# E3SM-Project/tinman_sandbox

Hardware: AMD Instinct MI355X
Metric: element-RHS-updates/sec (node) + achieved HBM GB/s, NP=4 NLEV=72 fp64 (higher is better)
Workload: dtype f64

## Files before the change

include/caar_tuning.h:

```cpp
#ifndef CAAR_TUNING_H
#define CAAR_TUNING_H

#include "caar.h"

#ifdef __cplusplus
extern "C" {
#endif

const char *caar_kernel_name(int np, int nlev);
int caar_num_variants(int np, int nlev);
int caar_select_variant(int np, int nlev, int variant);
int caar_selected_variant(int np, int nlev);
const char *caar_variant_info(int np, int nlev, int variant);
int caar_set_xcd_chunked(int on);
#define CAAR_CACHE_WINDOW_DEFAULT (224LL << 20)
int caar_set_cache_window(long long bytes);
long long caar_get_cache_window(void);
int caar_set_adaptive_window(int on);
int caar_get_adaptive_window(void);
long long caar_adaptive_window_lock_count(void);
int caar_adaptive_window_state(const double *vn0_dev, double *ms_window, double *ms_streaming, long long *probes);
int caar_adaptive_window_reset(void);


long long caar_context_cache_window(CaarContext *ctx);

int caar_set_fused_steps(int on);
int caar_get_fused_steps(void);
int caar_has_fused_steps(int np, int nlev, int variant);

enum { CAAR_PLACE_DEFAULT = 0, CAAR_PLACE_SPREAD = 1, CAAR_PLACE_MALLOC = 2 };
#define CAAR_PLACEMENT_POOL_DEFAULT (128LL << 30)
typedef struct CaarPlacement {
  int policy;
  long long pool_bytes;
  double max_free_fraction;
} CaarPlacement;
int caar_arrays_alloc_ex(CaarArena **arena, const CaarDims *dims, int device, const CaarPlacement *placement,
                         CaarArrays *out_dev);
int caar_arrays_placement(const CaarArena *arena, long long *pool_chunks, long long *chunk_bytes);

int caar_create_ex(CaarContext **ctx, const CaarDims *dims, int device, const CaarPlacement *placement);

int caar_stream_copy(double *dst_dev, const double *src_dev, long long n_doubles, int lane_bytes,
                     void *stream);
int caar_stream_copy_tuned(double *dst_dev, const double *src_dev, long long n_doubles, int variant,
                           void *stream);
int caar_stream_copy_tuned_variants(void);
const char *caar_stream_copy_tuned_info(int variant);
int caar_traffic_skeleton(const CaarDims *dims, const CaarArrays *dev, const CaarParams *params,
// ... 15 lines not shown
```

tinman_sandbox_amd/caar.py:

```python
import ctypes as C
import math
import os

import numpy as np
import torch

_HERE = os.path.dirname(os.path.abspath(__file__))
LIB_PATH = os.path.join(_HERE, "csrc", {"debug": "libcaar_hip_debug.so", "extra": "libcaar_hip_extra.so"}.get(
    os.environ.get("CAAR_LIBRARY", ""), "libcaar_hip.so"))
if os.environ.get("CAAR_LIBRARY_PATH"):
    LIB_PATH = os.environ["CAAR_LIBRARY_PATH"]

ARRAY_NAMES = (
    "elem_D", "elem_Dinv", "elem_fcor", "elem_spheremp", "elem_metdet", "elem_rmetdet",
    "elem_state_dp3d", "elem_state_v", "elem_state_T", "elem_state_phis", "elem_state_Qdp",
    "elem_derived_eta_dot_dpdn", "elem_derived_omega_p", "elem_derived_phi",
    "elem_derived_pecnd", "elem_derived_vn0",
)
MUTATED = ("elem_state_dp3d", "elem_state_v", "elem_state_T", "elem_derived_eta_dot_dpdn",
           "elem_derived_omega_p", "elem_derived_phi", "elem_derived_vn0")

_dp = C.POINTER(C.c_double)


# ... 33 lines not shown
class _CaarOperatorGeometry(C.Structure):
    _fields_ = [(n, C.c_void_p) for n in ("D", "Dinv", "metdet", "rmetdet", "spheremp", "mp", "metinv", "tensorVisc",
                                           "vec_sph2cart")]


class _CaarOperatorScalars(C.Structure):
    _fields_ = [("rrearth", C.c_double), ("alpha", C.c_double), ("beta", C.c_double), ("nu_ratio", C.c_double)]


SPHERE_OPERATORS = {
    "gradient_sphere": (0, False, True), "divergence_sphere": (1, True, False), "vorticity_sphere": (2, True, False),
    "divergence_sphere_wk": (3, True, False), "laplace_simple": (4, False, False), "laplace_tensor": (5, False, False),
    "curl_sphere_wk_testcov": (6, False, True), "grad_sphere_wk_testcov": (7, False, True),
    "vlaplace_sphere_wk_contra": (8, True, True), "vlaplace_sphere_wk_cartesian": (9, True, True),
    "gradient_sphere_update": (10, False, True), "divergence_sphere_update": (11, True, False),
    "vlaplace_sphere_wk_cartesian_damped": (12, True, True),
    "laplace_tensor_replace": (13, False, False),
}


class CaarLibrary:

    BOUNDARY_SYMBOLS = (
        "caar_supported", "caar_supported_ex", "caar_abi_version", "caar_device_count", "caar_strerror", "caar_array_len",
        "caar_algorithmic_bytes", "caar_launch", "caar_launch_steps", "caar_sphere_operator", "caar_sphere_operator_range",
        "caar_sphere_operator_ex", "caar_euler_step", "caar_preq_hydrostatic", "caar_preq_omega_ps", "caar_sphere_operator_host",
        "caar_preq_hydrostatic_host", "caar_preq_omega_ps_host", "caar_launch_state_norms", "caar_layout_from_f90",
        "caar_layout_to_f90", "caar_arrays_alloc", "caar_arrays_free", "caar_create", "caar_destroy", "caar_upload",
        "caar_download", "caar_upload_f90", "caar_download_f90", "caar_upload_f90_arrays", "caar_run", "caar_run_steps",
        "caar_sync", "caar_device_arrays", "caar_stream", "caar_state_norms", "caar_map_host", "caar_run_mapped",
        "caar_unmap_host")
    TUNING_SYMBOLS = (
        "caar_kernel_name", "caar_num_variants", "caar_select_variant", "caar_selected_variant", "caar_variant_info",
        "caar_set_xcd_chunked", "caar_set_cache_window", "caar_get_cache_window", "caar_set_adaptive_window",
        "caar_get_adaptive_window", "caar_adaptive_window_state", "caar_adaptive_window_reset", "caar_adaptive_window_lock_count",
        "caar_context_cache_window",
        "caar_set_fused_steps", "caar_get_fused_steps", "caar_has_fused_steps", "caar_arrays_alloc_ex",
        "caar_arrays_placement", "caar_create_ex", "caar_stream_copy", "caar_stream_copy_tuned",
        "caar_stream_copy_tuned_variants", "caar_stream_copy_tuned_info", "caar_traffic_skeleton", "caar_time_runs",
        "caar_reciprocal", "caar_debug_dp3d_violations")
    F90_SYMBOLS = ("caar_launch_f90", "caar_launch_steps_f90")
    DSS_SYMBOLS = ("caar_dss_plan_create", "caar_dss_plan_destroy", "caar_dss_plan_info", "caar_dss_launch")
    SYMBOLS = BOUNDARY_SYMBOLS + TUNING_SYMBOLS + F90_SYMBOLS + DSS_SYMBOLS

    def __init__(self, path=LIB_PATH):
        if not os.path.exists(path):
            raise CaarError(
                "HIP extension %s is missing: build it with `python -m tinman_sandbox_amd.build` "
                "(there is no CPU fallback)" % path)
        L = self.lib = C.CDLL(path)
        for s in self.SYMBOLS:
            getattr(L, s)
        vp = C.c_void_p
        L.caar_supported.argtypes = [C.c_int, C.c_int]
        L.caar_supported_ex.argtypes = [C.c_int, C.c_int, C.c_int]
        L.caar_debug_dp3d_violations.argtypes = [C.c_int]
        L.caar_debug_dp3d_violations.restype = C.c_longlong
        L.caar_strerror.argtypes = [C.c_int]
        L.caar_strerror.restype = C.c_char_p
        L.caar_array_len.argtypes = [C.POINTER(_CaarDims), C.c_int]
        L.caar_array_len.restype = C.c_longlong
        L.caar_algorithmic_bytes.argtypes = [C.c_int, C.c_int, C.c_int]
        L.caar_algorithmic_bytes.restype = C.c_longlong
        L.caar_launch.argtypes = [C.POINTER(_CaarDims), C.POINTER(_CaarArrays), vp,
                                  C.POINTER(_CaarParams), vp]
        L.caar_launch_steps.argtypes = [C.POINTER(_CaarDims), C.POINTER(_CaarArrays), vp, C.POINTER(_CaarParams), C.c_int,
                                        C.c_int, vp]
        L.caar_launch_f90.argtypes = [C.POINTER(_CaarDims), C.POINTER(_CaarArrays), vp, C.POINTER(_CaarParams), vp]
        L.caar_launch_steps_f90.argtypes = [C.POINTER(_CaarDims), C.POINTER(_CaarArrays), vp, C.POINTER(_CaarParams), C.c_int,
                                            C.c_int, vp]
        L.caar_launch_state_norms.argtypes = [C.POINTER(_CaarDims), C.POINTER(_CaarArrays), C.c_int,
                                              C.c_int, C.c_int, vp, vp]
        L.caar_sphere_operator.argtypes = [C.POINTER(_CaarDims), C.POINTER(_CaarArrays), vp, C.c_int, C.c_int,
                                           C.c_int, vp, vp, C.c_double, vp]
        L.caar_sphere_operator_range.argtypes = [C.POINTER(_CaarDims), C.POINTER(_CaarArrays), vp, C.c_int, C.c_int,
                                                 C.c_int, C.c_int, vp, vp, C.c_double, vp]
        L.caar_euler_step.argtypes = [C.POINTER(_CaarDims), C.POINTER(_CaarOperatorGeometry), vp, C.c_int, C.c_int, C.c_int,
                                      C.c_int, C.c_double, C.c_double, vp, vp, vp, vp]
        L.caar_sphere_operator_ex.argtypes = [C.POINTER(_CaarDims), C.POINTER(_CaarOperatorGeometry), vp, C.c_int, C.c_int,
                                              C.c_int, C.c_int, vp, vp, C.POINTER(_CaarOperatorScalars), vp]
        L.caar_preq_hydrostatic.argtypes = [C.POINTER(_CaarDims), C.c_int, vp, vp, vp, vp, C.c_double, vp, vp]
        L.caar_preq_omega_ps.argtypes = [C.POINTER(_CaarDims), C.c_int, vp, vp, vp, vp, vp]
        L.caar_sphere_operator_host.argtypes = [C.POINTER(_CaarDims), C.POINTER(_CaarArrays), vp, C.c_int, C.c_int, vp, vp,
                                                C.c_double]
        L.caar_preq_hydrostatic_host.argtypes = [C.POINTER(_CaarDims), vp, vp, vp, vp, C.c_double, vp]
        L.caar_preq_omega_ps_host.argtypes = [C.POINTER(_CaarDims), vp, vp, vp, vp]
        L.caar_reciprocal.argtypes = [vp, vp, C.c_longlong, vp]
        L.caar_kernel_name.argtypes = [C.c_int, C.c_int]
        L.caar_kernel_name.restype = C.c_char_p
        L.caar_num_variants.argtypes = [C.c_int, C.c_int]
        L.caar_select_variant.argtypes = [C.c_int, C.c_int, C.c_int]
        L.caar_variant_info.argtypes = [C.c_int, C.c_int, C.c_int]
        L.caar_variant_info.restype = C.c_char_p
        L.caar_set_xcd_chunked.argtypes = [C.c_int]
        L.caar_set_cache_window.argtypes = [C.c_longlong]
        L.caar_get_cache_window.restype = C.c_longlong
        L.caar_adaptive_window_state.argtypes = [vp, C.POINTER(C.c_double), C.POINTER(C.c_double), C.POINTER(C.c_longlong)]
        L.caar_adaptive_window_lock_count.restype = C.c_longlong
        L.caar_context_cache_window.argtypes = [vp]
        L.caar_context_cache_window.restype = C.c_longlong
        L.caar_selected_variant.argtypes = [C.c_int, C.c_int]
        L.caar_layout_from_f90.argtypes = [C.POINTER(_CaarDims), C.POINTER(_CaarArrays),
                                           C.POINTER(_CaarArrays), C.c_int, C.c_int, vp]
        L.caar_layout_to_f90.argtypes = [C.POINTER(_CaarDims), C.POINTER(_CaarArrays),
                                         C.POINTER(_CaarArrays), C.c_int, C.c_int, C.c_int, vp]
        L.caar_stream_copy.argtypes = [vp, vp, C.c_longlong, C.c_int, vp]
        L.caar_stream_copy_tuned.argtypes = [vp, vp, C.c_longlong, C.c_int, vp]
        L.caar_stream_copy_tuned_info.argtypes = [C.c_int]
        L.caar_stream_copy_tuned_info.restype = C.c_char_p
        L.caar_traffic_skeleton.argtypes = [C.POINTER(_CaarDims), C.POINTER(_CaarArrays),
                                            C.POINTER(_CaarParams), C.c_int, vp]
        L.caar_arrays_alloc.argtypes = [C.POINTER(vp), C.POINTER(_CaarDims), C.c_int, C.POINTER(_CaarArrays)]
        L.caar_arrays_alloc_ex.argtypes = [C.POINTER(vp), C.POINTER(_CaarDims), C.c_int, C.POINTER(_CaarPlacement),
                                           C.POINTER(_CaarArrays)]
        L.caar_arrays_free.argtypes = [vp]
        L.caar_arrays_placement.argtypes = [vp, C.POINTER(C.c_longlong), C.POINTER(C.c_longlong)]
        L.caar_create.argtypes = [C.POINTER(vp), C.POINTER(_CaarDims), C.c_int]
        L.caar_create_ex.argtypes = [C.POINTER(vp), C.POINTER(_CaarDims), C.c_int, C.POINTER(_CaarPlacement)]
        L.caar_destroy.argtypes = [vp]
        L.caar_destroy.restype = None
        L.caar_upload.argtypes = [vp, C.POINTER(_CaarArrays), C.c_int, C.c_int]
        L.caar_download.argtypes = [vp, C.POINTER(_CaarArrays), C.c_int, C.c_int, C.c_int]
        L.caar_upload_f90.argtypes = [vp, C.POINTER(_CaarArrays), C.c_int, C.c_int]
        L.caar_upload_f90_arrays.argtypes = [vp, C.POINTER(_CaarArrays), C.c_int, C.c_int, C.c_uint]
        L.caar_download_f90.argtypes = [vp, C.POINTER(_CaarArrays), C.c_int, C.c_int, C.c_int]
        L.caar_run.argtypes = [vp, C.POINTER(_CaarParams)]
        L.caar_sync.argtypes = [vp]
        L.caar_device_arrays.argtypes = [vp, C.POINTER(_CaarArrays)]
        L.caar_stream.argtypes = [vp]
# ... 594 lines not shown
```

tinman_sandbox_amd/csrc/caar_abi.hip:

```cpp
#include <hip/hip_runtime.h>

#include <atomic>
#include <cstdio>
#include <cstring>
#include <mutex>
#include <new>
#include <vector>

#include "../../include/caar.h"
#include "../../include/caar_f90.h"
#include "../../include/caar_tuning.h"
#include "caar_kernel_args.h"
#include "caar_window_tuner.h"

namespace caar {
extern KernelVariant kNp4Nlev72[];
extern int kNp4Nlev72Count;
extern KernelVariant kNp4Nlev128[];
extern int kNp4Nlev128Count;
extern KernelVariant kNp8Nlev72[];
extern int kNp8Nlev72Count;
#if CAAR_EXTRA_NLEV
extern KernelVariant kNp4Nlev32[], kNp4Nlev60[], kNp4Nlev64[], kNp4Nlev80[], kNp4Nlev96[], kNp4Nlev26[], kNp4Nlev30[];
extern int kNp4Nlev32Count, kNp4Nlev60Count, kNp4Nlev64Count, kNp4Nlev80Count, kNp4Nlev96Count, kNp4Nlev26Count, kNp4Nlev30Count;
// ... 81 lines not shown
  }
  void destroy() {
    if (dev) (void)hipFree(dev);
    delete host;
    dev = nullptr;
    host = nullptr;
  }
  hipError_t sync(const CaarDims& d, CaarParams* p, hipStream_t stream, const double** dvv_dev) {
    const size_t n = (size_t)d.np * d.np;
    if (!dvv_valid || std::memcmp(host->data(), p->Dvv, sizeof(double) * n) != 0) {
      std::memcpy(host->data(), p->Dvv, sizeof(double) * n);
      hipError_t e = hipMemcpyAsync(dev, host->data(), sizeof(double) * n, hipMemcpyHostToDevice, stream);
      if (e != hipSuccess) return e;
      dvv_valid = true;
    }
    if (p->rsplit == 0) {
      const size_t m = (size_t)d.nlev + 1;
      if (!hybi_valid || std::memcmp(host->data() + 64, p->hybi, sizeof(double) * m) != 0) {
        std::memcpy(host->data() + 64, p->hybi, sizeof(double) * m);
        hipError_t e = hipMemcpyAsync(dev + 64, host->data() + 64, sizeof(double) * m, hipMemcpyHostToDevice, stream);
        if (e != hipSuccess) return e;
        hybi_valid = true;
      }
      p->hybi_dev = dev + 64;
    }
    *dvv_dev = dev;
    return hipSuccess;
  }
};
}

static std::atomic<int> g_xcd_chunked{-1};
static std::atomic<long long> g_cache_window{CAAR_CACHE_WINDOW_DEFAULT};
static std::atomic<int> g_fused_steps{1};

namespace caar {
struct LaunchChoice {
  int variant;
  int xcd_chunked;
  long long cache_window;
  bool adapted;
};
static LaunchChoice launch_choice(const Config* cfg) {
  LaunchChoice c;
  c.variant = cfg ? cfg->selected.load(std::memory_order_relaxed) : 0;
  c.xcd_chunked = g_xcd_chunked.load(std::memory_order_relaxed);
  if (c.xcd_chunked < 0) c.xcd_chunked = cfg && cfg->variants[c.variant].prefers_xcd_chunked ? 1 : 0;
  c.cache_window = g_cache_window.load(std::memory_order_relaxed);
  c.adapted = false;
  return c;
}
}

namespace caar {
struct WindowTuner {
  std::atomic<const void*> key{nullptr};
  std::atomic<int> device{-1};
  std::atomic<int> use_window{1};
  std::atomic<long long> idle{0};
  WindowTunerState st;
  long long last_use = 0;
  hipEvent_t ev[WindowTunerState::kSlots] = {};

  void restart(const void* k, int dev) {
    key.store(nullptr, std::memory_order_relaxed);
    st.reset();
    last_use = 0;
    use_window.store(1, std::memory_order_relaxed);
    idle.store(0, std::memory_order_relaxed);
    device.store(dev, std::memory_order_relaxed);
    key.store(k, std::memory_order_release);
  }
};
struct HipStampBackend {
  WindowTuner* t;
  hipStream_t stream;
  bool stamp(int slot) {
    hipEvent_t& e = t->ev[slot];
    if (!e && hipEventCreate(&e) != hipSuccess) e = nullptr;
    return e && hipEventRecord(e, stream) == hipSuccess;
  }
// ... 150 lines not shown
  return (c->nlev != 0 || nlev <= 128 || CAAR_EXTRA_NLEV) ? 1 : 0;
}

const char* caar_kernel_name(int np, int nlev) {
  const caar::Config* c = caar::find_config(np, nlev);
  return c ? c->variants[c->selected.load()].kernel : nullptr;
}

int caar_num_variants(int np, int nlev) {
  const caar::Config* c = caar::find_config(np, nlev);
  return c ? c->count : 0;
}

int caar_select_variant(int np, int nlev, int variant) {
  caar::Config* c = caar::find_config(np, nlev);
  if (!c) return CAAR_EUNSUPPORTED;
  if (variant < 0 || variant >= c->count) return CAAR_EINVAL;
  c->selected.store(variant);
  return CAAR_OK;
}

int caar_selected_variant(int np, int nlev) {
  const caar::Config* c = caar::find_config(np, nlev);
  return c ? c->selected.load() : CAAR_EUNSUPPORTED;
}

int caar_set_cache_window(long long bytes) {
  if (bytes < 0) return CAAR_EINVAL;
  g_cache_window.store(bytes);
  return CAAR_OK;
}

long long caar_get_cache_window(void) { return g_cache_window.load(); }

int caar_set_adaptive_window(int on) {
  g_adaptive_window.store(on ? 1 : 0);
  return CAAR_OK;
}
int caar_get_adaptive_window(void) { return g_adaptive_window.load(); }

int caar_adaptive_window_state(const double* vn0_dev, double* ms_window, double* ms_streaming, long long* probes) {
  caar::WindowTuners* all = caar::window_tuners();
  std::lock_guard<std::mutex> g(all->mu);
  for (auto& t : all->t)
    if (vn0_dev && t.key.load(std::memory_order_relaxed) == (const void*)vn0_dev) {
      if (ms_window) *ms_window = t.st.ms_window;
      if (ms_streaming) *ms_streaming = t.st.ms_streaming;
      if (probes) *probes = t.st.probes;
      return t.use_window.load(std::memory_order_relaxed);
    }
  return -1;
}

long long caar_adaptive_window_lock_count(void) { return caar::window_tuners()->locked_calls.load(std::memory_order_relaxed); }

int caar_adaptive_window_reset(void) {
  caar::WindowTuners* all = caar::window_tuners();
  std::lock_guard<std::mutex> g(all->mu);
  for (auto& t : all->t) t.restart(nullptr, -1);
  return CAAR_OK;
}

int caar_set_fused_steps(int on) {
  g_fused_steps.store(on ? 1 : 0);
  return CAAR_OK;
}
// ... 562 lines not shown
  if (!out || !dims || dims->num_elems <= 0) return CAAR_EINVAL;
  if (!caar::find_config(dims->np, dims->nlev)) return CAAR_EUNSUPPORTED;
  int ndev = 0;
  if (hipGetDeviceCount(&ndev) != hipSuccess || ndev <= 0) return CAAR_ENODEVICE;
  if (device < 0 || device >= ndev) return CAAR_EINVAL;
  HIP_TRY(hipSetDevice(device));
  CaarContext* c = new (std::nothrow) CaarContext();
  if (!c) return CAAR_ENOMEM;
  std::memset(c, 0, sizeof(*c));
  c->dims = *dims;
  c->device = device;
  hipError_t e = hipStreamCreateWithFlags(&c->stream, hipStreamNonBlocking);
  if (e == hipSuccess) {
    const int rc = caar_arrays_alloc_ex(&c->arena, dims, device, placement, &c->dev);
    if (rc != CAAR_OK) {
      caar_destroy(c);
      return rc;
    }
  }
  if (e == hipSuccess) e = c->consts.create(dims->nlev);
  if (e == hipSuccess) e = hipMalloc((void**)&c->norms_dev, sizeof(double) * 3 * dims->num_elems);
  if (e != hipSuccess) {
    caar_destroy(c);
    return e == hipErrorOutOfMemory ? CAAR_ENOMEM : (int)e;
  }
  caar::device_shares_add(device, caar::keepable_bytes(c->dims));
  c->shares_registered = true;
  *out = c;
  return CAAR_OK;
}

long long caar_context_cache_window(CaarContext* c) {
  if (!c) return -1;
  return caar::device_share_of(c->device, c->dims, g_cache_window.load(std::memory_order_relaxed));
}

void caar_destroy(CaarContext* c) {
  if (!c) return;
  if (c->shares_registered) caar::device_shares_add(c->device, -caar::keepable_bytes(c->dims));
  int caller_dev = -1;
  if (hipGetDevice(&caller_dev) != hipSuccess) caller_dev = -1;
  (void)hipSetDevice(c->device);
  if (c->stream) (void)hipStreamSynchronize(c->stream);
  if (c->arena) (void)caar_arrays_free(c->arena);
  c->consts.destroy();
  if (c->norms_dev) (void)hipFree(c->norms_dev);
  if (c->stage_dev) (void)hipFree(c->stage_dev);
  if (c->steps_exec) (void)hipGraphExecDestroy(c->steps_exec);
  delete c->steps_hybi;
  if (c->stream) (void)hipStreamDestroy(c->stream);
  if (caller_dev >= 0 && caller_dev != c->device) (void)hipSetDevice(caller_dev);
  delete c;
}

static int copy_range(CaarContext* c, const CaarArrays* host, int i, int e0, int e1, bool to_device) {
  const long long per = caar_array_len(&c->dims, i) / c->dims.num_elems;
  double* h = *array_slot(host, i);
  double* d = *array_slot(&c->dev, i);
  if (!h) return CAAR_EINVAL;
  const size_t off = (size_t)per * e0, bytes = sizeof(double) * (size_t)per * (e1 - e0);
  if (to_device) HIP_TRY(hipMemcpyAsync(d + off, h + off, bytes, hipMemcpyHostToDevice, c->stream));
  else HIP_TRY(hipMemcpyAsync(h + off, d + off, bytes, hipMemcpyDeviceToHost, c->stream));
  return CAAR_OK;
}

int caar_upload(CaarContext* c, const CaarArrays* host, int e0, int e1) {
  if (!c || !host || e0 < 0 || e1 > c->dims.num_elems || e0 > e1) return CAAR_EINVAL;
// ... 302 lines not shown
```

tinman_sandbox_amd/csrc/caar_dss.hip:

```cpp
#include <hip/hip_runtime.h>

#include <algorithm>
#include <climits>
#include <cstdlib>
#include <new>
#include <utility>
#include <vector>

#include "../../include/caar_dss.h"

#pragma clang fp contract(off)

namespace caar {

constexpr int kDssThreads = 256;
constexpr int kDssLdsBytes = 32768;

__host__ __device__ constexpr int dss_bp_a(int np, int bp) {
  return bp < np ? 0 : (bp < np + 2 * (np - 2) ? 1 + (bp - np) / 2 : np - 1);
}
__host__ __device__ constexpr int dss_bp_b(int np, int bp) {
  return bp < np ? bp : (bp < np + 2 * (np - 2) ? (((bp - np) & 1) ? np - 1 : 0) : bp - np - 2 * (np - 2));
}
__host__ __device__ constexpr int dss_bp_of(int np, int a, int b) {
  return a == 0 ? b
                : (a == np - 1 ? np + 2 * (np - 2) + b
                               : (b == 0 ? np + 2 * (a - 1) : (b == np - 1 ? np + 2 * (a - 1) + 1 : -1)));
}

struct DssArgs {
  double* T;
  double* v;
  double* dp;
  const double* rsph;
  double* edge;
  const int* sharers;
  long long tstride;
  int nlev;
  int num_elems;
  int kc;
  int ldsw;
};

__device__ inline long long dss_element(int num_elems) {
  const int per = (num_elems + 7) / 8;
  const long long e = (long long)(blockIdx.x % 8) * per + blockIdx.x / 8;
  return e < num_elems ? e : -1;
}

template <int NP, bool F90>
__device__ inline double* dss_slab_value(const DssArgs& g, long long e, int k, int s, int& f, int& a, int& b) {
  constexpr int PP = NP * NP;
  const long long lev = e * g.tstride + (long long)k * PP;
  if (s < PP || s >= 3 * PP) {
    const int o = s < PP ? s : s - 3 * PP;
    f = s < PP ? 0 : 3;
    a = F90 ? o % NP : o / NP;
    b = F90 ? o / NP : o % NP;
    return (s < PP ? g.T : g.dp) + lev + o;
  }
  const int o = s - PP;
  int c, q;
  if (F90) {
    c = o / PP;
    q = o % PP;
    b = q / NP;
    a = q % NP;
  } else {
    c = o & 1;
    q = o >> 1;
    a = q / NP;
    b = q % NP;
  }
  f = 1 + c;
  return g.v + 2 * lev + o;
}

template <int NP, bool F90>
__device__ inline const double* dss_point(const DssArgs& g, long long e, int k, int f, int a, int b) {
  constexpr int PP = NP * NP;
  const long long lev = e * g.tstride + (long long)k * PP;
  const int p = F90 ? b * NP + a : a * NP + b;
  if (f == 0) return g.T + lev + p;
  if (f == 3) return g.dp + lev + p;
  return g.v + 2 * lev + (F90 ? (f - 1) * PP + p : 2 * p + (f - 1));
}

template <int NP, bool F90>
__global__ __launch_bounds__(kDssThreads) void caar_dss_pack(const DssArgs g) {
  constexpr int NB = 4 * (NP - 1);
  extern __shared__ double lds[];
  const long long e = dss_element(g.num_elems);
  if (e < 0) return;
  const int lane = threadIdx.x & 63, w = __builtin_amdgcn_readfirstlane(threadIdx.x >> 6);
  const int row4 = 4 * g.nlev, ldsw = g.ldsw;
  double* erow = g.edge + e * NB * row4;
  for (int k0 = 0; k0 < g.nlev; k0 += g.kc) {
    const int kc = min(g.kc, g.nlev - k0), n = kc * 4 * NB, m = 4 * kc;
#pragma unroll 4
    for (int i = threadIdx.x; i < n; i += kDssThreads) {
      const int kk = i / (4 * NB), r = i % (4 * NB), f = r / NB, bp = r % NB;
      lds[bp * ldsw + f * kc + kk] = *dss_point<NP, F90>(g, e, k0 + kk, f, dss_bp_a(NP, bp), dss_bp_b(NP, bp));
    }
    __syncthreads();
    for (int bp = w; bp < NB; bp += 4)
      for (int t = lane; t < m; t += 64) {
        const int f = t / kc;
        erow[bp * row4 + f * g.nlev + k0 + (t - f * kc)] = lds[bp * ldsw + t];
      }
    __syncthreads();
  }
}

template <int NP, bool F90>
__global__ __launch_bounds__(kDssThreads) void caar_dss_unpack(const DssArgs g) {
  constexpr int NB = 4 * (NP - 1), PP = NP * NP, MS = CAAR_DSS_MAX_SHARERS, BATCH = 8;
  extern __shared__ double lds[];
  const long long e = dss_element(g.num_elems);
  if (e < 0) return;
  const int lane = threadIdx.x & 63, w = __builtin_amdgcn_readfirstlane(threadIdx.x >> 6);
  const int row4 = 4 * g.nlev, ldsw = g.ldsw;
  const double* rsph = g.rsph + e * PP;
  for (int k0 = 0; k0 < g.nlev; k0 += g.kc) {
    const int kc = min(g.kc, g.nlev - k0), m = 4 * kc;
    for (int bp = w; bp < NB; bp += 4) {
      const int* sh = g.sharers + (e * NB + bp) * MS;
      int row[MS];
#pragma unroll
      for (int j = 0; j < MS; ++j) row[j] = sh[j];
      const int a = dss_bp_a(NP, bp), b = dss_bp_b(NP, bp);
      const double r = rsph[F90 ? b * NP + a : a * NP + b];
      for (int t0 = lane; t0 < m; t0 += 128) {
        double x[2][MS];
#pragma unroll
        for (int q = 0; q < 2; ++q) {
          const int t = t0 + 64 * q, f = t / kc;
          const long long col = (long long)f * g.nlev + k0 + (t - f * kc);
#pragma unroll
          for (int j = 0; j < MS; ++j)
            if (t < m && row[j] >= 0) x[q][j] = g.edge[(long long)row[j] * row4 + col];
        }
#pragma unroll
        for (int q = 0; q < 2; ++q) {
          const int t = t0 + 64 * q;
          if (t < m) {
            double S = x[q][0];
#pragma unroll
            for (int j = 1; j < MS; ++j)
              if (row[j] >= 0) S = S + x[q][j];
            lds[bp * ldsw + t] = r * S;
          }
        }
      }
    }
    __syncthreads();
    const int n = kc * 4 * PP;
    for (int b0 = threadIdx.x; b0 < n; b0 += BATCH * kDssThreads) {
      double v[BATCH];
#pragma unroll
      for (int q = 0; q < BATCH; ++q) {
        const int i = b0 + q * kDssThreads, kk = i / (4 * PP), s = i % (4 * PP);
        int f, a, b;
        const double* p = dss_slab_value<NP, F90>(g, e, k0 + kk, s, f, a, b);
        if (i < n && dss_bp_of(NP, a, b) < 0) v[q] = *p;
      }
#pragma unroll
      for (int q = 0; q < BATCH; ++q) {
        const int i = b0 + q * kDssThreads, kk = i / (4 * PP), s = i % (4 * PP);
        int f, a, b;
        double* p = dss_slab_value<NP, F90>(g, e, k0 + kk, s, f, a, b);
        const int bp = dss_bp_of(NP, a, b);
        if (i < n) *p = bp >= 0 ? lds[bp * ldsw + f * kc + kk] : rsph[F90 ? b * NP + a : a * NP + b] * v[q];
      }
    }
    __syncthreads();
  }
}

template <int NP, bool F90>
static hipError_t launch_dss(const DssArgs& g, int num_elems, hipStream_t stream) {
  const int grid = 8 * ((num_elems + 7) / 8);
  const size_t lds = sizeof(double) * 4 * (NP - 1) * g.ldsw;
  hipLaunchKernelGGL((caar_dss_pack<NP, F90>), dim3(grid), dim3(kDssThreads), lds, stream, g);
  hipError_t e = hipGetLastError();
  if (e != hipSuccess) return e;
  hipLaunchKernelGGL((caar_dss_unpack<NP, F90>), dim3(grid), dim3(kDssThreads), lds, stream, g);
  return hipGetLastError();
}

}

struct CaarDssPlan {
  int np, nlev, num_elems, layout, device;
  long long unique_points, shared_points, open_points;
  int max_sharers;
  int* rows_dev;
  double* edge_dev;
};

namespace {

int dss_analyse(CaarDssPlan* P, const long long* gdof, std::vector<int>& rows) {
  const int NP = P->np, PP = NP * NP, NB = 4 * (NP - 1);
  const long long NE = P->num_elems, npts = NE * PP;
  std::vector<long long> g((size_t)npts);
  for (long long e = 0; e < NE; ++e)
    for (int a = 0; a < NP; ++a)
      for (int b = 0; b < NP; ++b) {
        const long long id = gdof[e * PP + (P->layout == CAAR_DSS_LAYOUT_F90 ? b * NP + a : a * NP + b)];
        if (id < 0) return CAAR_EINVAL;
        g[(size_t)(e * PP + a * NP + b)] = id;
      }
  std::vector<int> order((size_t)npts);
  for (long long i = 0; i < npts; ++i) order[(size_t)i] = (int)i;
  std::sort(order.begin(), order.end(), [&](int x, int y) { return g[x] != g[y] ? g[x] < g[y] : x < y; });
// ... 70 lines not shown
}

}

extern "C" {

int caar_dss_plan_create(CaarDssPlan** plan, const CaarDims* dims, const long long* gdof_host, int layout, int device) {
  if (!plan) return CAAR_EINVAL;
  *plan = nullptr;
  if (!dims || (dims->num_elems > 0 && !gdof_host)) return CAAR_EINVAL;
  if (layout != CAAR_DSS_LAYOUT_CXX && layout != CAAR_DSS_LAYOUT_F90) return CAAR_EINVAL;
  if (dims->num_elems < 0) return CAAR_EINVAL;
  if ((dims->np != 4 && dims->np != 8) || !caar_supported(dims->np, dims->nlev)) return CAAR_EUNSUPPORTED;
  const int NB = 4 * (dims->np - 1);
  if ((long long)dims->num_elems * NB * CAAR_DSS_MAX_SHARERS >= INT_MAX) return CAAR_EINVAL;
  CaarDssPlan* P = new (std::nothrow) CaarDssPlan();
  if (!P) return CAAR_ENOMEM;
  P->np = dims->np;
  P->nlev = dims->nlev;
  P->num_elems = dims->num_elems;
  P->layout = layout;
  P->device = device < 0 ? -1 : device;
  std::vector<int> rows;
  int rc;
  try {
    rc = dss_analyse(P, gdof_host, rows);
  } catch (const std::bad_alloc&) {
    rc = CAAR_ENOMEM;
  }
  if (rc == CAAR_OK && P->device >= 0) {
    int caller = -1;
    hipError_t e = hipGetDevice(&caller);
    if (e == hipSuccess) e = hipSetDevice(P->device);
    const size_t edge_n = (size_t)P->num_elems * NB * 4 * P->nlev;
    if (e == hipSuccess) e = hipMalloc((void**)&P->rows_dev, sizeof(int) * std::max<size_t>(rows.size(), 1));
    if (e == hipSuccess) e = hipMalloc((void**)&P->edge_dev, sizeof(double) * std::max<size_t>(edge_n, 1));
    if (e == hipSuccess && !rows.empty())
      e = hipMemcpy(P->rows_dev, rows.data(), sizeof(int) * rows.size(), hipMemcpyHostToDevice);
    if (caller >= 0 && caller != P->device) (void)hipSetDevice(caller);
    if (e != hipSuccess) rc = e == hipErrorOutOfMemory ? CAAR_ENOMEM : (int)e;
  }
  if (rc != CAAR_OK) {
    dss_free_device(P);
    delete P;
    return rc;
  }
  *plan = P;
  return CAAR_OK;
}

void caar_dss_plan_destroy(CaarDssPlan* plan) {
  if (!plan) return;
  dss_free_device(plan);
  delete plan;
}

int caar_dss_plan_info(const CaarDssPlan* plan, long long* unique_points, long long* shared_points, long long* open_points,
                       int* max_sharers) {
  if (!plan) return CAAR_EINVAL;
  if (unique_points) *unique_points = plan->unique_points;
  if (shared_points) *shared_points = plan->shared_points;
  if (open_points) *open_points = plan->open_points;
  if (max_sharers) *max_sharers = plan->max_sharers;
  return CAAR_OK;
}

int caar_dss_launch(const CaarDssPlan* plan, const CaarDims* dims, int layout, const CaarArrays* arrays_dev, int tl,
                    const double* rspheremp_dev, void* stream) {
  if (!plan || !dims || !arrays_dev || !rspheremp_dev) return CAAR_EINVAL;
  if (dims->np != plan->np || dims->nlev != plan->nlev || dims->num_elems != plan->num_elems || dims->timelevels < 1)
    return CAAR_EINVAL;
  if (layout != plan->layout || tl < 0 || tl >= dims->timelevels) return CAAR_EINVAL;
  double* T = arrays_dev->elem_state_T;
  double* v = arrays_dev->elem_state_v;
  double* dp = arrays_dev->elem_state_dp3d;
  if (!T || !v || !dp) return CAAR_EINVAL;
  if (((size_t)T | (size_t)v | (size_t)dp | (size_t)rspheremp_dev) & 7) return CAAR_EINVAL;
  if (plan->device < 0) return CAAR_ENODEVICE;
  if (plan->num_elems == 0) return CAAR_OK;
  const long long pp = (long long)plan->np * plan->np, lev = (long long)plan->nlev * pp;
  caar::DssArgs g;
  g.T = T + tl * lev;
  g.v = v + 2 * tl * lev;
  g.dp = dp + tl * lev;
  g.rsph = rspheremp_dev;
  g.edge = plan->edge_dev;
  g.sharers = plan->rows_dev;
  g.tstride = (long long)dims->timelevels * lev;
  g.nlev = plan->nlev;
  g.num_elems = plan->num_elems;
  const int nb = 4 * (plan->np - 1), kc_max = (caar::kDssLdsBytes / (8 * nb) - 1) / 4;
  const int passes = (plan->nlev + kc_max - 1) / kc_max;
  g.kc = (plan->nlev + passes - 1) / passes;
  g.ldsw = 4 * g.kc + 1;
  const hipStream_t s = (hipStream_t)stream;
  hipError_t e;
  if (plan->np == 4)
    e = plan->layout == CAAR_DSS_LAYOUT_F90 ? caar::launch_dss<4, true>(g, plan->num_elems, s)
                                            : caar::launch_dss<4, false>(g, plan->num_elems, s);
  else
    e = plan->layout == CAAR_DSS_LAYOUT_F90 ? caar::launch_dss<8, true>(g, plan->num_elems, s)
                                            : caar::launch_dss<8, false>(g, plan->num_elems, s);
  return (int)e;
}

}
```

tinman_sandbox_amd/csrc/caar_kernel_args.h:

```cpp
#pragma once

#include <hip/hip_runtime.h>

#ifndef CAAR_EXTRA_NLEV
#define CAAR_EXTRA_NLEV 0
#endif

namespace caar {

struct KernelArgs {
  const double* D;
  const double* Dinv;
  const double* fcor;
  const double* spheremp;
  const double* metdet;
  const double* rmetdet;
  double* dp3d;
  double* v;
  double* T;
  const double* phis;
  const double* Qdp;
  double* eta_dot_dpdn;
  double* omega_p;
  double* phi;
  const double* pecnd;
  double* vn0;
  const double* Dvv;
  const double* hybi;
  int vadv;
  int nets;
  int nelem;
  int per_xcd;
  unsigned cache_q_lo, cache_q_hi;
  int n0, np1, nm1;
  int qn0;
  int qsize_d, timelevels;
  int nlev;
  double dt2;
  double rrearth;
  double eta_ave_w;
  double rv_over_rd_m1;
  double Rgas;
  double kappa;
  double p_top;
};

__device__ __forceinline__ long long element_of_block(const KernelArgs& k, unsigned b) {
  if (k.per_xcd == 0) return (long long)k.nets + b;
  const unsigned x = b & 7u, s = b >> 3;
  const unsigned e = x * (unsigned)k.per_xcd + s;
  return (s < (unsigned)k.per_xcd && e < (unsigned)k.nelem) ? (long long)k.nets + e : -1;
}

__device__ __forceinline__ void request_kernel_args(const KernelArgs& k) {
  asm volatile("" ::"s"(k.D), "s"(k.v), "s"(k.vn0), "s"(k.timelevels));
}

__device__ __forceinline__ bool element_is_cached(const KernelArgs& k, long long ie) {
  const unsigned long long q = ((unsigned long long)k.cache_q_hi << 32) | k.cache_q_lo;
  const unsigned long long e = (unsigned long long)ie;
  return (((e + 1) * q) >> 32) > ((e * q) >> 32);
}

__device__ __forceinline__ double recip(double x) {
  double r = __builtin_amdgcn_rcp(x);
  double e = __builtin_fma(-x, r, 1.0);
  r = __builtin_fma(r, e, r);
  e = __builtin_fma(-x, r, 1.0);
  r = __builtin_fma(r, e, r);
  return r;
}

__device__ __forceinline__ double dot2(double a, double b, double c, double d) { return __builtin_fma(a, b, c * d); }


typedef double dbl2 __attribute__((ext_vector_type(2)));
template <bool NT, typename T>
__device__ __forceinline__ T stream_load(const T* p) {
  if constexpr (NT) return __builtin_nontemporal_load(p);
  else return *p;
}
template <bool NT, typename T>
__device__ __forceinline__ void stream_store(T* p, T v) {
  if constexpr (NT) __builtin_nontemporal_store(v, p);
  else *p = v;
}

template <bool NT, int PLANE>
__device__ __forceinline__ dbl2 f90_pair_load(const dbl2* base, unsigned i) {
  const double* p = reinterpret_cast<const double*>(base) + i;
  dbl2 x;
  x.x = stream_load<NT>(p);
  x.y = stream_load<NT>(p + PLANE);
  return x;
// ... 77 lines not shown
```

Before: 32.85 million.

## Rewrite DSS pack/unpack with register-resident slabs, vector edge rows and cache-share policy

Rewrites the DSS pack and unpack kernels so each thread loads its slice of T/v/dp once into registers with optional 16-byte vector nontemporal loads. It scatters boundary points to LDS and stores the whole slab back in one pass, replacing per-point index decoding and the separate interior re-read. The edge buffer rows are padded and laid out for dbl2 access. Pack and unpack walk elements in opposite orders. A new tunable DSS cache share subtracts from the CAAR cache window and marks some edge rows for temporal stores. Occupancy hints are added, at the cost of more register pressure and a more complex indexing scheme.

```diff
diff --git a/include/caar_tuning.h b/include/caar_tuning.h
--- a/include/caar_tuning.h
+++ b/include/caar_tuning.h
@@ -16,6 +16,9 @@
 #define CAAR_CACHE_WINDOW_DEFAULT (224LL << 20)
 int caar_set_cache_window(long long bytes);
 long long caar_get_cache_window(void);
+#define CAAR_DSS_CACHE_SHARE_DEFAULT 0LL
+int caar_set_dss_cache_share(long long bytes);
+long long caar_get_dss_cache_share(void);
 int caar_set_adaptive_window(int on);
 int caar_get_adaptive_window(void);
 long long caar_adaptive_window_lock_count(void);
diff --git a/tinman_sandbox_amd/caar.py b/tinman_sandbox_amd/caar.py
--- a/tinman_sandbox_amd/caar.py
+++ b/tinman_sandbox_amd/caar.py
@@ -89,7 +89,8 @@
         "caar_unmap_host")
     TUNING_SYMBOLS = (
         "caar_kernel_name", "caar_num_variants", "caar_select_variant", "caar_selected_variant", "caar_variant_info",
-        "caar_set_xcd_chunked", "caar_set_cache_window", "caar_get_cache_window", "caar_set_adaptive_window",
+        "caar_set_xcd_chunked", "caar_set_cache_window", "caar_get_cache_window", "caar_set_dss_cache_share",
+        "caar_get_dss_cache_share", "caar_set_adaptive_window",
         "caar_get_adaptive_window", "caar_adaptive_window_state", "caar_adaptive_window_reset", "caar_adaptive_window_lock_count",
         "caar_context_cache_window",
         "caar_set_fused_steps", "caar_get_fused_steps", "caar_has_fused_steps", "caar_arrays_alloc_ex",
@@ -152,6 +153,8 @@
         L.caar_set_xcd_chunked.argtypes = [C.c_int]
         L.caar_set_cache_window.argtypes = [C.c_longlong]
         L.caar_get_cache_window.restype = C.c_longlong
+        L.caar_set_dss_cache_share.argtypes = [C.c_longlong]
+        L.caar_get_dss_cache_share.restype = C.c_longlong
         L.caar_adaptive_window_state.argtypes = [vp, C.POINTER(C.c_double), C.POINTER(C.c_double), C.POINTER(C.c_longlong)]
         L.caar_adaptive_window_lock_count.restype = C.c_longlong
         L.caar_context_cache_window.argtypes = [vp]
diff --git a/tinman_sandbox_amd/csrc/caar_abi.hip b/tinman_sandbox_amd/csrc/caar_abi.hip
--- a/tinman_sandbox_amd/csrc/caar_abi.hip
+++ b/tinman_sandbox_amd/csrc/caar_abi.hip
@@ -137,6 +137,11 @@
 
 static std::atomic<int> g_xcd_chunked{-1};
 static std::atomic<long long> g_cache_window{CAAR_CACHE_WINDOW_DEFAULT};
+static std::atomic<long long> g_dss_cache_share{CAAR_DSS_CACHE_SHARE_DEFAULT};
+static long long routine_cache_window() {
+  const long long w = g_cache_window.load(std::memory_order_relaxed) - g_dss_cache_share.load(std::memory_order_relaxed);
+  return w > 0 ? w : 0;
+}
 static std::atomic<int> g_fused_steps{1};
 
 namespace caar {
@@ -151,7 +156,7 @@
   c.variant = cfg ? cfg->selected.load(std::memory_order_relaxed) : 0;
   c.xcd_chunked = g_xcd_chunked.load(std::memory_order_relaxed);
   if (c.xcd_chunked < 0) c.xcd_chunked = cfg && cfg->variants[c.variant].prefers_xcd_chunked ? 1 : 0;
-  c.cache_window = g_cache_window.load(std::memory_order_relaxed);
+  c.cache_window = routine_cache_window();
   c.adapted = false;
   return c;
 }
@@ -368,6 +373,14 @@
 }
 
 long long caar_get_cache_window(void) { return g_cache_window.load(); }
+
+int caar_set_dss_cache_share(long long bytes) {
+  if (bytes < 0) return CAAR_EINVAL;
+  g_dss_cache_share.store(bytes);
+  return CAAR_OK;
+}
+
+long long caar_get_dss_cache_share(void) { return g_dss_cache_share.load(); }
 
 int caar_set_adaptive_window(int on) {
   g_adaptive_window.store(on ? 1 : 0);
@@ -996,7 +1009,7 @@
 
 long long caar_context_cache_window(CaarContext* c) {
   if (!c) return -1;
-  return caar::device_share_of(c->device, c->dims, g_cache_window.load(std::memory_order_relaxed));
+  return caar::device_share_of(c->device, c->dims, routine_cache_window());
 }
 
 void caar_destroy(CaarContext* c) {
diff --git a/tinman_sandbox_amd/csrc/caar_dss.hip b/tinman_sandbox_amd/csrc/caar_dss.hip
--- a/tinman_sandbox_amd/csrc/caar_dss.hip
+++ b/tinman_sandbox_amd/csrc/caar_dss.hip
@@ -8,6 +8,8 @@
 #include <vector>
 
 #include "../../include/caar_dss.h"
+#include "../../include/caar_tuning.h"
+#include "caar_kernel_args.h"
 
 #pragma clang fp contract(off)
 
@@ -15,6 +17,17 @@
 
 constexpr int kDssThreads = 256;
 constexpr int kDssLdsBytes = 32768;
+__host__ __device__ constexpr int dss_kc_max(int np) { return ((kDssLdsBytes / (8 * 4 * (np - 1)) - 1) / 4) & ~1; }
+__host__ __device__ constexpr int dss_units_t(int np) { return (dss_kc_max(np) * np * np / 2 + kDssThreads - 1) / kDssThreads; }
+__host__ __device__ constexpr int dss_pass_levels(int np, int nlev) {
+  const int passes = (nlev + dss_kc_max(np) - 1) / dss_kc_max(np);
+  return ((nlev + passes - 1) / passes + 1) & ~1;
+}
+__host__ __device__ constexpr int dss_row_doubles(int np, int nlev) {
+  const int kc = dss_pass_levels(np, nlev);
+  return (nlev + kc - 1) / kc * 4 * kc;
+}
+__host__ __device__ constexpr int dss_slots(int np) { return 2 * 4 * dss_units_t(np); }
 
 __host__ __device__ constexpr int dss_bp_a(int np, int bp) {
   return bp < np ? 0 : (bp < np + 2 * (np - 2) ? 1 + (bp - np) / 2 : np - 1);
@@ -37,150 +50,243 @@
   const int* sharers;
   long long tstride;
   int nlev;
+  int rowlen;
   int num_elems;
   int kc;
   int ldsw;
+  int wide;
+  unsigned keep_q_lo, keep_q_hi;
 };
 
+template <bool DESCENDING>
 __device__ inline long long dss_element(int num_elems) {
-  const int per = (num_elems + 7) / 8;
-  const long long e = (long long)(blockIdx.x % 8) * per + blockIdx.x / 8;
+  const int per = (num_elems + 7) / 8, s = blockIdx.x / 8;
+  const long long e = (long long)(blockIdx.x % 8) * per + (DESCENDING ? per - 1 - s : s);
   return e < num_elems ? e : -1;
 }
 
-template <int NP, bool F90>
-__device__ inline double* dss_slab_value(const DssArgs& g, long long e, int k, int s, int& f, int& a, int& b) {
-  constexpr int PP = NP * NP;
-  const long long lev = e * g.tstride + (long long)k * PP;
-  if (s < PP || s >= 3 * PP) {
-    const int o = s < PP ? s : s - 3 * PP;
-    f = s < PP ? 0 : 3;
-    a = F90 ? o % NP : o / NP;
-    b = F90 ? o / NP : o % NP;
-    return (s < PP ? g.T : g.dp) + lev + o;
-  }
-  const int o = s - PP;
-  int c, q;
-  if (F90) {
-    c = o / PP;
-    q = o % PP;
-    b = q / NP;
-    a = q % NP;
-  } else {
-    c = o & 1;
-    q = o >> 1;
-    a = q / NP;
-    b = q % NP;
-  }
-  f = 1 + c;
-  return g.v + 2 * lev + o;
-}
-
-template <int NP, bool F90>
-__device__ inline const double* dss_point(const DssArgs& g, long long e, int k, int f, int a, int b) {
-  constexpr int PP = NP * NP;
-  const long long lev = e * g.tstride + (long long)k * PP;
-  const int p = F90 ? b * NP + a : a * NP + b;
-  if (f == 0) return g.T + lev + p;
-  if (f == 3) return g.dp + lev + p;
-  return g.v + 2 * lev + (F90 ? (f - 1) * PP + p : 2 * p + (f - 1));
-}
-
-template <int NP, bool F90>
-__global__ __launch_bounds__(kDssThreads) void caar_dss_pack(const DssArgs g) {
+__device__ __forceinline__ bool dss_row_kept(const DssArgs& g, long long ie) {
+  return element_is_cached_q(((unsigned long long)g.keep_q_hi << 32) | g.keep_q_lo, ie);
+}
+
+template <int NP, bool F90, bool WIDE>
+struct DssPass {
+  static constexpr int PP = NP * NP, UT = dss_units_t(NP), S = dss_slots(NP);
+  double *T, *v, *dp;
+  unsigned nT;
+  unsigned tid;
+  int bptab;
+  __device__ __forceinline__ DssPass(const DssArgs& g, long long e, int k0, int kc) {
+    const long long lev = e * g.tstride + (long long)k0 * PP;
+    T = g.T + lev;
+    v = g.v + 2 * lev;
+    dp = g.dp + lev;
+    nT = kc * PP;
+    tid = threadIdx.x;
+    forget_places();
+    const int pl = tid & (PP - 1);
+    bptab = dss_bp_of(NP, F90 ? pl % NP : pl / NP, F90 ? pl / NP : pl % NP);
+  }
+  __device__ __forceinline__ void forget_places() { asm volatile("" : "+v"(tid)); }
+  static __device__ __forceinline__ constexpr int run_of(int s) { return (s >> 1) < UT ? 0 : ((s >> 1) < 3 * UT ? 1 : 2); }
+  __device__ __forceinline__ unsigned offset(int s) const {
+    const unsigned run = run_of(s), u = (s >> 1) - (run == 0 ? 0 : (run == 1 ? UT : 3 * UT));
+    return WIDE ? 2 * (tid + kDssThreads * u) + (s & 1) : tid + kDssThreads * (2 * u + (s & 1));
+  }
+  __device__ __forceinline__ bool valid(int s) const { return offset(s) < (run_of(s) == 1 ? 2 * nT : nT); }
+  __device__ __forceinline__ double* address(int s) const {
+    return (run_of(s) == 0 ? T : (run_of(s) == 1 ? v : dp)) + offset(s);
+  }
+  __device__ __forceinline__ void decode(int s, int& f, int& kk, int& p, int& bp) const {
+    const unsigned o = offset(s);
+    if (run_of(s) != 1) {
+      f = run_of(s) == 0 ? 0 : 3;
+      kk = o / PP;
+      p = o % PP;
+    } else {
+      const unsigned q = o % (2 * PP);
+      kk = o / (2 * PP);
+      p = F90 ? q % PP : q >> 1;
+      f = 1 + (F90 ? q / PP : q & 1);
+    }
+    bp = __shfl(bptab, p);
+  }
+
+  __device__ __forceinline__ void load(double (&x)[S]) const {
+#pragma unroll
+    for (int s = 0; s < S; ++s) x[s] = 0.0;
+    if constexpr (WIDE) {
+#pragma unroll
+      for (int s = 0; s < S; s += 2)
+        if (valid(s)) {
+          const dbl2 t = stream_load<true>(reinterpret_cast<const dbl2*>(address(s)));
+          x[s] = t.x;
+          x[s + 1] = t.y;
+        }
+    } else {
+#pragma unroll
+      for (int s = 0; s < S; ++s)
+        if (valid(s)) x[s] = stream_load<true>(address(s));
+    }
+  }
+  __device__ __forceinline__ void store(const double (&x)[S]) const {
+    if constexpr (WIDE) {
+#pragma unroll
+      for (int s = 0; s < S; s += 2)
+        if (valid(s)) {
+          dbl2 t;
+          t.x = x[s];
+          t.y = x[s + 1];
+          stream_store<true>(reinterpret_cast<dbl2*>(address(s)), t);
+        }
+    } else {
+#pragma unroll
+      for (int s = 0; s < S; ++s)
+        if (valid(s)) stream_store<true>(address(s), x[s]);
+    }
+  }
+  __device__ __forceinline__ void boundary_to_lds(const DssArgs& g, double* lds, const double (&x)[S]) const {
+#pragma unroll
+    for (int s = 0; s < S; ++s) {
+      lds[image_place(g, s)] = x[s];
+    }
+  }
+  __device__ __forceinline__ int image_place(const DssArgs& g, int s) const {
+    int f, kk, p, bp;
+    decode(s, f, kk, p, bp);
+    return valid(s) && bp >= 0 ? bp * g.ldsw + f * g.kc + kk : 4 * (NP - 1) * g.ldsw;
+  }
+};
+
+template <int NP, bool F90, bool WIDE>
+__device__ __forceinline__ void dss_pack_body(const DssArgs& g, long long e, double* lds) {
   constexpr int NB = 4 * (NP - 1);
-  extern __shared__ double lds[];
-  const long long e = dss_element(g.num_elems);
-  if (e < 0) return;
   const int lane = threadIdx.x & 63, w = __builtin_amdgcn_readfirstlane(threadIdx.x >> 6);
-  const int row4 = 4 * g.nlev, ldsw = g.ldsw;
-  double* erow = g.edge + e * NB * row4;
+  dbl2* erow = reinterpret_cast<dbl2*>(g.edge + e * NB * g.rowlen);
+  const bool keep = dss_row_kept(g, e);
   for (int k0 = 0; k0 < g.nlev; k0 += g.kc) {
-    const int kc = min(g.kc, g.nlev - k0), n = kc * 4 * NB, m = 4 * kc;
-#pragma unroll 4
-    for (int i = threadIdx.x; i < n; i += kDssThreads) {
-      const int kk = i / (4 * NB), r = i % (4 * NB), f = r / NB, bp = r % NB;
-      lds[bp * ldsw + f * kc + kk] = *dss_point<NP, F90>(g, e, k0 + kk, f, dss_bp_a(NP, bp), dss_bp_b(NP, bp));
-    }
+    const int kc = min(g.kc, g.nlev - k0);
+    const DssPass<NP, F90, WIDE> ps(g, e, k0, kc);
+    double x[dss_slots(NP)];
+    ps.load(x);
+    ps.boundary_to_lds(g, lds, x);
     __syncthreads();
     for (int bp = w; bp < NB; bp += 4)
-      for (int t = lane; t < m; t += 64) {
-        const int f = t / kc;
-        erow[bp * row4 + f * g.nlev + k0 + (t - f * kc)] = lds[bp * ldsw + t];
+      for (int t2 = lane; t2 < 2 * g.kc; t2 += 64) {
+        dbl2 val;
+        val.x = lds[bp * g.ldsw + 2 * t2];
+        val.y = lds[bp * g.ldsw + 2 * t2 + 1];
+        dbl2* dst = erow + ((bp * g.rowlen + 4 * k0) >> 1) + t2;
+        if (keep) stream_store<false>(dst, val);
+        else stream_store<true>(dst, val);
       }
     __syncthreads();
   }
 }
 
 template <int NP, bool F90>
-__global__ __launch_bounds__(kDssThreads) void caar_dss_unpack(const DssArgs g) {
-  constexpr int NB = 4 * (NP - 1), PP = NP * NP, MS = CAAR_DSS_MAX_SHARERS, BATCH = 8;
+__global__ __launch_bounds__(kDssThreads) __attribute__((amdgpu_waves_per_eu(NP == 4 ? 5 : 3))) void caar_dss_pack(const DssArgs g) {
   extern __shared__ double lds[];
-  const long long e = dss_element(g.num_elems);
+  const long long e = dss_element<true>(g.num_elems);
   if (e < 0) return;
+  if (g.wide) dss_pack_body<NP, F90, true>(g, e, lds);
+  else dss_pack_body<NP, F90, false>(g, e, lds);
+}
+
+template <int NP, bool F90, bool WIDE>
+__device__ __forceinline__ void dss_unpack_body(const DssArgs& g, long long e, double* lds) {
+  constexpr int NB = 4 * (NP - 1), PP = NP * NP, MS = CAAR_DSS_MAX_SHARERS, GRP = 2;
+  constexpr int CH = (2 * dss_kc_max(NP) + 63) / 64;
   const int lane = threadIdx.x & 63, w = __builtin_amdgcn_readfirstlane(threadIdx.x >> 6);
-  const int row4 = 4 * g.nlev, ldsw = g.ldsw;
   const double* rsph = g.rsph + e * PP;
+  const dbl2* edge = reinterpret_cast<const dbl2*>(g.edge);
   for (int k0 = 0; k0 < g.nlev; k0 += g.kc) {
-    const int kc = min(g.kc, g.nlev - k0), m = 4 * kc;
+    const int kc = min(g.kc, g.nlev - k0);
+    DssPass<NP, F90, WIDE> ps(g, e, k0, kc);
+    double x[dss_slots(NP)];
+    ps.load(x);
+    const double rlane = rsph[ps.tid & (PP - 1)];
+    ps.boundary_to_lds(g, lds, x);
+#pragma unroll
+    for (int s = 0; s < dss_slots(NP); ++s) {
+      int f, kk, p, bp;
+      ps.decode(s, f, kk, p, bp);
+      x[s] = __shfl(rlane, p) * x[s];
+    }
+    ps.forget_places();
+    __syncthreads();
     for (int bp = w; bp < NB; bp += 4) {
-      const int* sh = g.sharers + (e * NB + bp) * MS;
+      const int self = (int)e * NB + bp;
+      const int* sh = g.sharers + (long long)self * MS;
       int row[MS];
 #pragma unroll
-      for (int j = 0; j < MS; ++j) row[j] = sh[j];
+      for (int j = 0; j < MS; ++j) row[j] = __builtin_amdgcn_readfirstlane(sh[j]);
       const int a = dss_bp_a(NP, bp), b = dss_bp_b(NP, bp);
       const double r = rsph[F90 ? b * NP + a : a * NP + b];
-      for (int t0 = lane; t0 < m; t0 += 128) {
-        double x[2][MS];
-#pragma unroll
-        for (int q = 0; q < 2; ++q) {
-          const int t = t0 + 64 * q, f = t / kc;
-          const long long col = (long long)f * g.nlev + k0 + (t - f * kc);
-#pragma unroll
-          for (int j = 0; j < MS; ++j)
-            if (t < m && row[j] >= 0) x[q][j] = g.edge[(long long)row[j] * row4 + col];
+      dbl2 S[CH];
+#pragma unroll
+      for (int j0 = 0; j0 < MS; j0 += GRP) {
+        if (row[j0] < 0) break;
+        dbl2 y[CH][GRP];
+#pragma unroll
+        for (int j = 0; j < GRP; ++j)
+          if (row[j0 + j] >= 0 && row[j0 + j] != self) {
+            const bool kept = dss_row_kept(g, row[j0 + j] / NB);
+            const dbl2* src = edge + (((long long)row[j0 + j] * g.rowlen + 4 * k0) >> 1);
+#pragma unroll
+            for (int c = 0; c < CH; ++c)
+              if (lane + 64 * c < 2 * g.kc)
+                y[c][j] = kept ? stream_load<false>(src + (lane + 64 * c)) : stream_load<true>(src + (lane + 64 * c));
+          }
+#pragma unroll
+        for (int c = 0; c < CH; ++c)
+          if (lane + 64 * c < 2 * g.kc) {
+            const double* img = lds + bp * g.ldsw + 2 * (lane + 64 * c);
+            dbl2 own;
+            own.x = img[0];
+            own.y = img[1];
+#pragma unroll
+            for (int j = 0; j < GRP; ++j)
+              if (row[j0 + j] >= 0) {
+                const dbl2 term = row[j0 + j] == self ? own : y[c][j];
+                S[c] = j0 + j == 0 ? term : S[c] + term;
+              }
+          }
+      }
+#pragma unroll
+      for (int c = 0; c < CH; ++c)
+        if (lane + 64 * c < 2 * g.kc) {
+          double* img = lds + bp * g.ldsw + 2 * (lane + 64 * c);
+          img[0] = r * S[c].x;
+          img[1] = r * S[c].y;
         }
-#pragma unroll
-        for (int q = 0; q < 2; ++q) {
-          const int t = t0 + 64 * q;
-          if (t < m) {
-            double S = x[q][0];
-#pragma unroll
-            for (int j = 1; j < MS; ++j)
-              if (row[j] >= 0) S = S + x[q][j];
-            lds[bp * ldsw + t] = r * S;
-          }
-        }
-      }
     }
     __syncthreads();
-    const int n = kc * 4 * PP;
-    for (int b0 = threadIdx.x; b0 < n; b0 += BATCH * kDssThreads) {
-      double v[BATCH];
-#pragma unroll
-      for (int q = 0; q < BATCH; ++q) {
-        const int i = b0 + q * kDssThreads, kk = i / (4 * PP), s = i % (4 * PP);
-        int f, a, b;
-        const double* p = dss_slab_value<NP, F90>(g, e, k0 + kk, s, f, a, b);
-        if (i < n && dss_bp_of(NP, a, b) < 0) v[q] = *p;
-      }
-#pragma unroll
-      for (int q = 0; q < BATCH; ++q) {
-        const int i = b0 + q * kDssThreads, kk = i / (4 * PP), s = i % (4 * PP);
-        int f, a, b;
-        double* p = dss_slab_value<NP, F90>(g, e, k0 + kk, s, f, a, b);
-        const int bp = dss_bp_of(NP, a, b);
-        if (i < n) *p = bp >= 0 ? lds[bp * ldsw + f * kc + kk] : rsph[F90 ? b * NP + a : a * NP + b] * v[q];
-      }
-    }
+    ps.forget_places();
+#pragma unroll
+    for (int s = 0; s < dss_slots(NP); ++s) {
+      const int at = ps.image_place(g, s);
+      const double y = lds[at];
+      x[s] = at < NB * g.ldsw ? y : x[s];
+    }
+    ps.store(x);
     __syncthreads();
   }
+}
+
+template <int NP, bool F90>
+__global__ __launch_bounds__(kDssThreads) __attribute__((amdgpu_waves_per_eu(NP == 4 ? 4 : 2))) void caar_dss_unpack(const DssArgs g) {
+  extern __shared__ double lds[];
+  const long long e = dss_element<false>(g.num_elems);
+  if (e < 0) return;
+  if (g.wide) dss_unpack_body<NP, F90, true>(g, e, lds);
+  else dss_unpack_body<NP, F90, false>(g, e, lds);
 }
 
 template <int NP, bool F90>
 static hipError_t launch_dss(const DssArgs& g, int num_elems, hipStream_t stream) {
   const int grid = 8 * ((num_elems + 7) / 8);
-  const size_t lds = sizeof(double) * 4 * (NP - 1) * g.ldsw;
+  const size_t lds = sizeof(double) * (4 * (NP - 1) * g.ldsw + 1);
   hipLaunchKernelGGL((caar_dss_pack<NP, F90>), dim3(grid), dim3(kDssThreads), lds, stream, g);
   hipError_t e = hipGetLastError();
   if (e != hipSuccess) return e;
@@ -317,7 +423,7 @@
     int caller = -1;
     hipError_t e = hipGetDevice(&caller);
     if (e == hipSuccess) e = hipSetDevice(P->device);
-    const size_t edge_n = (size_t)P->num_elems * NB * 4 * P->nlev;
+    const size_t edge_n = (size_t)P->num_elems * NB * caar::dss_row_doubles(P->np, P->nlev);
     if (e == hipSuccess) e = hipMalloc((void**)&P->rows_dev, sizeof(int) * std::max<size_t>(rows.size(), 1));
     if (e == hipSuccess) e = hipMalloc((void**)&P->edge_dev, sizeof(double) * std::max<size_t>(edge_n, 1));
     if (e == hipSuccess && !rows.empty())
@@ -374,10 +480,19 @@
   g.tstride = (long long)dims->timelevels * lev;
   g.nlev = plan->nlev;
   g.num_elems = plan->num_elems;
-  const int nb = 4 * (plan->np - 1), kc_max = (caar::kDssLdsBytes / (8 * nb) - 1) / 4;
-  const int passes = (plan->nlev + kc_max - 1) / kc_max;
-  g.kc = (plan->nlev + passes - 1) / passes;
+  g.wide = ((((size_t)g.T | (size_t)g.v | (size_t)g.dp) & 15) == 0) ? 1 : 0;
+  const int nb = 4 * (plan->np - 1);
+  g.kc = caar::dss_pass_levels(plan->np, plan->nlev);
   g.ldsw = 4 * g.kc + 1;
+  g.rowlen = caar::dss_row_doubles(plan->np, plan->nlev);
+  {
+    const long long share = std::min(caar_get_dss_cache_share(), caar_get_cache_window());
+    const long long per_elem = 8LL * nb * g.rowlen;
+    const long long count = std::min<long long>(share / per_elem, plan->num_elems);
+    const unsigned long long q = ((unsigned long long)count << 32) / (unsigned long long)plan->num_elems;
+    g.keep_q_lo = (unsigned)(q & 0xffffffffull);
+    g.keep_q_hi = (unsigned)(q >> 32);
+  }
   const hipStream_t s = (hipStream_t)stream;
   hipError_t e;
   if (plan->np == 4)
diff --git a/tinman_sandbox_amd/csrc/caar_kernel_args.h b/tinman_sandbox_amd/csrc/caar_kernel_args.h
--- a/tinman_sandbox_amd/csrc/caar_kernel_args.h
+++ b/tinman_sandbox_amd/csrc/caar_kernel_args.h
@@ -56,10 +56,12 @@
   asm volatile("" ::"s"(k.D), "s"(k.v), "s"(k.vn0), "s"(k.timelevels));
 }
 
-__device__ __forceinline__ bool element_is_cached(const KernelArgs& k, long long ie) {
-  const unsigned long long q = ((unsigned long long)k.cache_q_hi << 32) | k.cache_q_lo;
+__device__ __forceinline__ bool element_is_cached_q(unsigned long long q, long long ie) {
   const unsigned long long e = (unsigned long long)ie;
   return (((e + 1) * q) >> 32) > ((e * q) >> 32);
+}
+__device__ __forceinline__ bool element_is_cached(const KernelArgs& k, long long ie) {
+  return element_is_cached_q(((unsigned long long)k.cache_q_hi << 32) | k.cache_q_lo, ie);
 }
 
 __device__ __forceinline__ double recip(double x) {
```

Result: no change. 32.81 million (-0.1%).
